# Sagnac/OpticalRayTracing.jl

Measured on NVIDIA B200. Metric: FP64 ray-surface intersections/sec, higher is better.
Workload: dtype f64

## Files before the change

### opticalraytracing.jl_b200/csrc/kern_trace3d.cu

```cuda
#include "kern.cuh"

struct Hit {
    double xs, ys;
    double xf, yf;
    unsigned flags;
    double opl;
};

__device__ __forceinline__ double strict_opl_start(const RayS& r, int mode, double n0, double y, double x, double z0)
{
    if (mode == 1) return SD(SM(n0, -z0), r.k3);
    return SM(n0, SA(SM(x, r.k1), SM(y, r.k2)));
}

__device__ __forceinline__ double strict_opl_close(const RayS& r, const ort_field& f, double nlast)
{
    if (f.opd_radius == 0.0) return r.opl;
    const double qx = SS(r.x, f.opd_xc), qy = SS(r.y, f.opd_yc);
    const double b = SA(SM(qx, r.k1), SM(qy, r.k2));
    const double cq = SS(SA(SM(qx, qx), SM(qy, qy)), SM(f.opd_radius, f.opd_radius));
    const double sg = (f.opd_radius < 0.0) ? -1.0 : 1.0;
    const double tau = SS(-b, SM(sg, SQ(SS(SM(b, b), cq))));
    return SA(r.opl, SM(nlast, tau));
}

template <bool EXT, class SurfArray, bool POLY, bool XF>
__device__ __forceinline__ Hit trace_strict_impl(const SurfArray& S, int nsurf, int stop, double y, double x, double u, double v,
                                                 const ort_field* fld, double n0, double nlast, bool vignette, const double* poly,
                                                 int npoly, int* bad)
{
    RayS r;
    strict_init<XF>(r, y, x, u, v);
    if (EXT) r.opl = strict_opl_start(r, fld->mode, n0, y, x, fld->z0);
    Hit h; h.xs = h.ys = CUDART_NAN; h.opl = 0.0;
    for (int i = 0; i < nsurf; i++) {
        strict_step<EXT, POLY, XF>(S[i], r, vignette, (POLY && poly) ? poly + (size_t)i * npoly : nullptr, npoly);
        if (i == stop - 1) { h.xs = r.x; h.ys = r.y; }
    }
    h.xf = r.x; h.yf = r.y; h.flags = r.flags;
    if (EXT) h.opl = strict_opl_close(r, *fld, nlast);
    if (XF) *bad = r.bad;
    return h;
}

template <bool EXT, class SurfArray, bool POLY = false>
__device__ __forceinline__ Hit trace_strict(const SurfArray& S, int nsurf, int stop,
                                            double y, double x, double u, double v,
                                            const ort_field* fld = nullptr, double n0 = 1.0, double nlast = 1.0,
                                            bool vignette = false, const double* poly = nullptr, int npoly = 0)
{
    return trace_strict_impl<EXT, SurfArray, POLY, false>(S, nsurf, stop, y, x, u, v, fld, n0, nlast, vignette, poly, npoly, nullptr);
}

template <bool EXT, class SurfArray, bool POLY = false>
__device__ __noinline__ Hit trace_strict_cold(const SurfArray& S, int nsurf, int stop,
                                              double y, double x, double u, double v,
                                              const ort_field* fld = nullptr, double n0 = 1.0, double nlast = 1.0,
                                              bool vignette = false, const double* poly = nullptr, int npoly = 0)
{
    return trace_strict<EXT, SurfArray, POLY>(S, nsurf, stop, y, x, u, v, fld, n0, nlast, vignette, poly, npoly);
}

template <bool EXT, class SurfArray, bool POLY = false>
__device__ __forceinline__ Hit trace_strict_xf(const SurfArray& S, int nsurf, int stop,
                                               double y, double x, double u, double v,
                                               const ort_field* fld = nullptr, double n0 = 1.0, double nlast = 1.0,
                                               bool vignette = false, const double* poly = nullptr, int npoly = 0)
{
    int bad = 0;
    const Hit h = trace_strict_impl<EXT, SurfArray, POLY, true>(S, nsurf, stop, y, x, u, v, fld, n0, nlast, vignette, poly, npoly, &bad);
    if (bad) return trace_strict_cold<EXT, SurfArray, POLY>(S, nsurf, stop, y, x, u, v, fld, n0, nlast, vignette, poly, npoly);
    return h;
}

__device__ __forceinline__ int nonfinite_bit(double a) { return 0x7FEFFFFF - (hi32(a) & 0x7FFFFFFF); }

__device__ __forceinline__ bool is_nan_bits(double a)
{
    return (hi32(a) & 0x7FFFFFFF) > 0x7FF00000 ||
           ((hi32(a) & 0x7FFFFFFF) == 0x7FF00000 && __double2loint(a) != 0);
}

template <int RPT, bool EXT, class SurfArray, bool MIRROR = true, int SIMPLE = 0, bool R2ONLY = false, int POLY = 0, class QT = NoPolyK>
__device__ __forceinline__ void trace_fast(const SurfArray& S, int nsurf, int stop, double n0,
                                           const double* y, const double* x, const double* u,
                                           const double* v, Hit* h, int* amb,
                                           const ort_field* fld = nullptr, double nlast = 1.0, bool vignette = false,
                                           const double* K0 = nullptr, bool kzcheck = true, const double* poly = nullptr,
                                           int npoly = 0, const QT* Q = nullptr)
{
    RaysF<RPT> r;
#pragma unroll
    for (int j = 0; j < RPT; j++) {
        if (K0) {
            r.x[j] = x[j]; r.y[j] = y[j]; r.z[j] = 0.0;
            r.Kx[j] = K0[0]; r.Ky[j] = K0[1]; r.Kz[j] = K0[2];
            r.amb[j] = 0; r.opl[j] = 0.0; r.vig[j] = 0;
        } else fast_init(r, j, n0, y[j], x[j], u[j], v[j]);
        if (EXT) {
            r.opl[j] = (fld->mode == 1) ? fast_div(-(n0 * n0) * fld->z0, r.Kz[j]) : fma(x[j], r.Kx[j], y[j] * r.Ky[j]);
        }
    }
    int i = 0;
    for (; i < stop; i++)
        if constexpr (POLY == 2) fast_step<RPT, EXT, MIRROR, SIMPLE, 2>(S[i], r, vignette, nullptr, 0, 0, &Q->r[i]);
        else fast_step<RPT, EXT, MIRROR, SIMPLE, POLY>(S[i], r, vignette, (POLY && poly) ? poly + (size_t)i * npoly : nullptr, npoly, nsurf * npoly);
#pragma unroll
    for (int j = 0; j < RPT; j++) {
        if (R2ONLY) { h[j].xs = fma(r.x[j], r.x[j], r.y[j] * r.y[j]); h[j].ys = 0.0; }
        else { h[j].xs = r.x[j]; h[j].ys = r.y[j]; }
    }
    for (; i < nsurf; i++)
        if constexpr (POLY == 2) fast_step<RPT, EXT, MIRROR, SIMPLE, 2>(S[i], r, vignette, nullptr, 0, 0, &Q->r[i]);
        else fast_step<RPT, EXT, MIRROR, SIMPLE, POLY>(S[i], r, vignette, (POLY && poly) ? poly + (size_t)i * npoly : nullptr, npoly, nsurf * npoly);
#pragma unroll
    for (int j = 0; j < RPT; j++) {
        h[j].xf = r.x[j]; h[j].yf = r.y[j];
        h[j].flags = (EXT && r.vig[j]) ? ORT_FLAG_VIGN : 0u;
        amb[j] = r.amb[j] | nonfinite_bit(r.x[j]) | nonfinite_bit(r.y[j]);
        if (kzcheck) amb[j] |= nonfinite_bit(r.Kz[j]);
        h[j].opl = 0.0;
        if (EXT) {
            double opl = r.opl[j];
            if (fld->opd_radius != 0.0) {
                const double qx = r.x[j] - fld->opd_xc, qy = r.y[j] - fld->opd_yc;
                const double bK = fma(qx, r.Kx[j], qy * r.Ky[j]);
                const double cq = fma(qx, qx, fma(qy, qy, -fld->opd_radius * fld->opd_radius));
                const double d = fma(bK, bK, -(nlast * nlast) * cq);
                double sq = fast_sqrt(d);
                if ((fld->opd_radius < 0.0) != (nlast < 0.0)) sq = -sq;
                opl = opl - bK - sq;
                amb[j] |= nonfinite_bit(opl);
            }
            h[j].opl = opl;
        }
    }
}

struct RawAcc {
    int n, nflag_lo, nflag_hi;
    double s1x, s2x, s1y, s2y, rmax;
    double s1o, s2o; int nvig;
    int nstrict;
};

__device__ __forceinline__ void raw_add(RawPart& p, const RawPart& q)
{
    p.n += q.n; p.s1x += q.s1x; p.s2x += q.s2x; p.s1y += q.s1y; p.s2y += q.s2y;
    p.rmax = fmax(p.rmax, q.rmax);
    p.nmiss += q.nmiss; p.ntir += q.ntir; p.ndom += q.ndom; p.nclip += q.nclip;
    p.s1o += q.s1o; p.s2o += q.s2o; p.nvig += q.nvig; p.nstrict += q.nstrict;
}

__device__ __forceinline__ void raw_warp_reduce(RawPart& p)
{
#pragma unroll
    for (int d = 16; d >= 1; d >>= 1) {
        p.n += __shfl_down_sync(0xffffffffu, p.n, d);
        p.s1x += __shfl_down_sync(0xffffffffu, p.s1x, d);
        p.s2x += __shfl_down_sync(0xffffffffu, p.s2x, d);
        p.s1y += __shfl_down_sync(0xffffffffu, p.s1y, d);
        p.s2y += __shfl_down_sync(0xffffffffu, p.s2y, d);
        p.rmax = fmax(p.rmax, __shfl_down_sync(0xffffffffu, p.rmax, d));
        p.nmiss += __shfl_down_sync(0xffffffffu, p.nmiss, d);
        p.ntir += __shfl_down_sync(0xffffffffu, p.ntir, d);
        p.ndom += __shfl_down_sync(0xffffffffu, p.ndom, d);
        p.nclip += __shfl_down_sync(0xffffffffu, p.nclip, d);
        p.s1o += __shfl_down_sync(0xffffffffu, p.s1o, d);
        p.s2o += __shfl_down_sync(0xffffffffu, p.s2o, d);
        p.nvig += __shfl_down_sync(0xffffffffu, p.nvig, d);
        p.nstrict += __shfl_down_sync(0xffffffffu, p.nstrict, d);
    }
}

template <int NWARPS>
__device__ __forceinline__ void raw_block_reduce(RawPart& p, RawPart* smem )
{
    raw_warp_reduce(p);
    const int lane = threadIdx.x & 31, warp = threadIdx.x >> 5;
    if (lane == 0) smem[warp] = p;
    __syncthreads();
    if (threadIdx.x == 0)
        for (int w = 1; w < NWARPS; w++) raw_add(p, smem[w]);
}

__device__ __forceinline__ void field_slopes(const ort_field& fld, double y0, double x0, double& u, double& v)
{
    u = fld.u; v = fld.v;
    if (fld.mode == 1) {
        u = tan(SD(SS(fld.ybar, y0), fld.z0));
        v = tan(SD(-x0, fld.z0));
    }
}

struct LeanPtrs { double *ex, *ey, *opd; uint8_t* mask; };
template <int ARITH, int EXTK, int LEAN, bool R2ONLY = false, int POLYK = 0>
__device__ __forceinline__ int grid_epilogue(const Presc& P, const GridArgs& A, const ort_field& fld,
                                             const double* ysf, Hit h, int amb, unsigned idx,
                                             bool valid, size_t fbase, double cx, double cy, double co, RawAcc& acc,
                                             const LeanPtrs& lp)
{
    constexpr bool EXT = EXTK != 0;
    const size_t o = fbase + idx;
    const bool vignette = EXTK == 1 && (A.ext & ORT_EXT_VIGNETTE);
    double ri = 0.0, r2 = 0.0;
    bool clip = false;
    if (ARITH == ORT_ARITH_FAST) {
        r2 = R2ONLY ? h.xs : fma(h.xs, h.xs, h.ys * h.ys);
        amb |= tiny_vs_bit(r2 - A.a_stop2, A.a_stop2);
        clip = r2 > A.a_stop2;
    }
    const bool sv = (ARITH == ORT_ARITH_STRICT) || amb < 0;
    if (sv) {
        if (ARITH != ORT_ARITH_STRICT) {
            const unsigned iy = idx / (unsigned)A.nx, ix = idx - iy * (unsigned)A.nx;
            const double y0 = __ldg(ysf + iy), x0 = __ldg(A.xs + ix);
            double u, v; field_slopes(fld, y0, x0, u, v);
            h = trace_strict_cold<EXT, decltype(P.s), POLYK != 0>(P.s, P.nsurf, A.stop, y0, x0, u, v, &fld, P.n0, P.nlast, vignette, P.poly, P.npoly);
        }
        ri = jl_hypot(h.xs, h.ys);
        clip = ri > A.a_stop;
        r2 = ri * ri;
        if (valid) {
            acc.nstrict++;
            acc.nflag_lo += (h.flags & ORT_FLAG_MISS ? 1 : 0) + (h.flags & ORT_FLAG_TIR ? 0x10000 : 0);
            acc.nflag_hi += (h.flags & ORT_FLAG_DOMAIN ? 1 : 0);
        }
    } else if (!LEAN && A.r) {
        ri = (r2 > 0.0) ? fast_sqrt(r2) : r2;
    }
    const bool vig = EXTK == 1 && (h.flags & ORT_FLAG_VIGN);
    const bool drop = clip || vig || (sv && (is_nan_bits(h.xf) || is_nan_bits(h.yf)));
    const unsigned flags = h.flags | (clip ? ORT_FLAG_CLIP : 0u);
    const int kept = valid && !drop;
    const double ex = h.xf;
    const double ey = SS(h.yf, fld.h_prime);
    double opd = 0.0;
    if (EXT && (A.ext & ORT_EXT_OPD)) opd = SM(SS(h.opl, fld.opl_ref), A.opd_scale);
    if (LEAN) {
        if (valid) {
            if (LEAN == 1) { *lp.ex = ex; *lp.ey = ey; *lp.mask = (uint8_t)kept; }
            if (LEAN == 1 && EXT) *lp.opd = opd;
            if (EXTK == 1) acc.nvig += vig ? 1 : 0;
            if (clip) acc.nflag_hi += 0x10000;
        }
    } else if (valid) {
        if (A.ex) A.ex[o] = ex;
        if (A.ey) A.ey[o] = ey;
        if (A.r) A.r[o] = ri;
        if (A.theta) A.theta[o] = atan2(h.ys, h.xs);
        if (A.wx) A.wx[o] = SD(SM(ex, A.wg_nu), A.wg_lambda);
        if (A.wy) A.wy[o] = SD(SM(ey, A.wg_nu), A.wg_lambda);
        if (EXT && A.opd) A.opd[o] = opd;
        if (A.mask) A.mask[o] = (uint8_t)kept;
        if (A.flags) A.flags[o] = (uint8_t)flags;
        acc.nflag_hi += clip ? 0x10000 : 0;
        if (EXT) acc.nvig += vig ? 1 : 0;
    }
    if (kept) {
        const double dx = ex - cx, dy = ey - cy;
        acc.s1x += dx; acc.s2x = fma(dx, dx, acc.s2x);
        acc.s1y += dy; acc.s2y = fma(dy, dy, acc.s2y);
        { const double rv = (ARITH == ORT_ARITH_STRICT) ? ri : r2; if (rv > acc.rmax) acc.rmax = rv; }
        if (EXT) { const double dd = opd - co; acc.s1o += dd; acc.s2o = fma(dd, dd, acc.s2o); }
        acc.n++;
    }
    return kept;
}

template <int ARITH, int RPT, int EXTK, int LEAN = 0, bool MIRROR = true, int SIMPLE = 0, int POLYK = 0>
__global__ void __launch_bounds__(ORT_TILE, (ARITH == ORT_ARITH_FAST) ? POLYK ? ORT_BPS_POLY : (SIMPLE == 2 ? ORT_BPSC : SIMPLE ? (EXTK ? ORT_BPSE : ORT_BPSP) : (RPT == 1 ? ORT_BPS1 : (EXTK ? ORT_BPS2E : ORT_BPS2))) : ORT_BPSS)
k_grid(const __grid_constant__ Presc P, const __grid_constant__ GridArgs A, const __grid_constant__ typename PolyArg<POLYK>::type Q)
{
    constexpr bool EXT = EXTK != 0;
    __shared__ RawPart s_part[ORT_TILE / 32];
    __shared__ double s_shift[3];
    const int f = blockIdx.y;
    const ort_field& fld = A.fields[f];
    const unsigned NN = A.NN;
    const unsigned nsub = (NN + ORT_TILE - 1) / ORT_TILE;
    const unsigned ntiles = (nsub + RPT - 1) / RPT;
    const size_t fbase = (size_t)f * NN;
    const double* ysf = A.ys + (size_t)f * A.ys_stride;
    const unsigned ysoff = (unsigned)f * (unsigned)A.ys_stride;
    const bool vignette = EXTK == 1 && (A.ext & ORT_EXT_VIGNETTE);

    RawAcc acc;
    acc.n = acc.nflag_lo = acc.nflag_hi = acc.nvig = acc.nstrict = 0;
    acc.s1x = acc.s2x = acc.s1y = acc.s2y = acc.s1o = acc.s2o = 0.0; acc.rmax = -CUDART_INF;

    if (threadIdx.x == 0) {
        const double y0 = __ldg(ysf + A.ny / 2), x0 = __ldg(A.xs);
        double u, v; field_slopes(fld, y0, x0, u, v);
        Hit h; int amb = 0;
        if (ARITH == ORT_ARITH_FAST)
            trace_fast<1, EXT, decltype(P.s), SIMPLE == 0, SIMPLE, false, POLYK, typename PolyArg<POLYK>::type>(P.s, P.nsurf, A.stop, P.n0, &y0, &x0, &u, &v, &h, &amb, &fld, P.nlast, vignette,
                                                                   nullptr, true, P.poly, P.npoly, &Q);
        if (ARITH == ORT_ARITH_STRICT || amb < 0)
            h = trace_strict_cold<EXT, decltype(P.s), (EXT && ARITH == ORT_ARITH_STRICT) || POLYK != 0>(P.s, P.nsurf, A.stop, y0, x0, u, v, &fld, P.n0,
                                                                                                  P.nlast, vignette, P.poly, P.npoly);
        const double ey = h.yf - fld.h_prime;
        const bool bad = nonfinite_bit(h.xf) < 0 || nonfinite_bit(ey) < 0;
        s_shift[0] = bad ? 0.0 : h.xf;
        s_shift[1] = bad ? 0.0 : ey;
        const double od = (h.opl - fld.opl_ref) * A.opd_scale;
        s_shift[2] = (!EXT || !(A.ext & ORT_EXT_OPD) || bad || nonfinite_bit(od) < 0) ? 0.0 : od;
    }
    __syncthreads();
    const double cx = s_shift[0], cy = s_shift[1], co = s_shift[2];
    constexpr bool R2ONLY = ARITH == ORT_ARITH_FAST && LEAN != 0;
    const bool kzcheck = P.s[P.nsurf - 1].kcode != SURF_PLANE;

    const bool collimated = (fld.mode == 0);
    double K0[3] = {0.0, 0.0, 0.0};
    if (ARITH == ORT_ARITH_FAST && collimated) {
        const double inv = P.n0 * fast_rsqrt(fma(fld.v, fld.v, fma(fld.u, fld.u, 1.0)));
        K0[0] = fld.v * inv; K0[1] = fld.u * inv; K0[2] = inv;
    }
    const unsigned nxu = (unsigned)A.nx;
    const unsigned step = gridDim.x * (RPT * ORT_TILE);
    const unsigned dq = step / nxu, dr = step - dq * nxu;
    unsigned iyj[RPT], ixj[RPT];
#pragma unroll
    for (int j = 0; j < RPT; j++) {
        const unsigned i0 = (blockIdx.x * RPT + j) * ORT_TILE + threadIdx.x;
        iyj[j] = i0 / nxu; ixj[j] = i0 - iyj[j] * nxu;
    }

    for (unsigned tile = blockIdx.x; tile < ntiles; tile += gridDim.x) {
        double y0[RPT], x0[RPT], u[RPT], v[RPT];
        unsigned idx[RPT];
        bool valid[RPT];
#pragma unroll
        for (int j = 0; j < RPT; j++) {
            const unsigned i0 = (tile * RPT + j) * ORT_TILE + threadIdx.x;
            valid[j] = i0 < NN;
            idx[j] = min(i0, NN - 1);
            const unsigned iy = min(iyj[j], (unsigned)A.ny - 1), ix = ixj[j];
            y0[j] = __ldg(A.ys + (ysoff + iy)); x0[j] = __ldg(A.xs + ix);
            u[j] = 0.0; v[j] = 0.0;
            ixj[j] += dr; iyj[j] += dq;
            if (ixj[j] >= nxu) { ixj[j] -= nxu; iyj[j]++; }
        }
        if (!collimated || ARITH != ORT_ARITH_FAST) {
#pragma unroll
            for (int j = 0; j < RPT; j++) field_slopes(fld, y0[j], x0[j], u[j], v[j]);
        }
        Hit h[RPT];
        int amb[RPT];
        if (ARITH == ORT_ARITH_FAST)
            trace_fast<RPT, EXT, decltype(P.s), MIRROR, SIMPLE, R2ONLY, POLYK, typename PolyArg<POLYK>::type>(P.s, P.nsurf, A.stop, P.n0, y0, x0, u, v, h, amb, &fld, P.nlast, vignette,
                                                                collimated ? K0 : nullptr, kzcheck, P.poly, P.npoly, &Q);
        else {
            RayS r[RPT];
#pragma unroll
            for (int j = 0; j < RPT; j++) {
                strict_init<ORT_STRICT_XF>(r[j], y0[j], x0[j], u[j], v[j]);
                if (EXT) r[j].opl = strict_opl_start(r[j], fld.mode, P.n0, y0[j], x0[j], fld.z0);
                h[j].xs = h[j].ys = CUDART_NAN; h[j].opl = 0.0;
            }
            const int nsurf = P.nsurf, stop = A.stop;
            for (int i = 0; i < nsurf; i++) {
#pragma unroll
                for (int j = 0; j < RPT; j++) {
                    strict_step<EXT, EXT, ORT_STRICT_XF>(P.s[i], r[j], vignette, (EXT && P.poly) ? P.poly + (size_t)i * P.npoly : nullptr, P.npoly);
                    if (i == stop - 1) { h[j].xs = r[j].x; h[j].ys = r[j].y; }
                }
            }
#pragma unroll
            for (int j = 0; j < RPT; j++) {
                h[j].xf = r[j].x; h[j].yf = r[j].y; h[j].flags = r[j].flags;
                if (EXT) h[j].opl = strict_opl_close(r[j], fld, P.nlast);
                if (ORT_STRICT_XF && r[j].bad)
                    h[j] = trace_strict_cold<EXT, decltype(P.s), EXT>(P.s, P.nsurf, A.stop, y0[j], x0[j], u[j], v[j], &fld, P.n0, P.nlast, vignette, P.poly, P.npoly);
            }
        }
        int keptj[RPT];
        LeanPtrs lp0 = {nullptr, nullptr, nullptr, nullptr};
        if (LEAN == 1) {
            const size_t e0 = fbase + (size_t)tile * (RPT * ORT_TILE) + threadIdx.x;
            lp0.ex = A.ex + e0; lp0.ey = A.ey + e0; lp0.mask = A.mask + e0;
            if (EXT) lp0.opd = A.opd + e0;
        }
#pragma unroll
        for (int j = 0; j < RPT; j++) {
            if (ARITH != ORT_ARITH_FAST) amb[j] = 0;
            const LeanPtrs lp = {lp0.ex + j * ORT_TILE, lp0.ey + j * ORT_TILE, EXT ? lp0.opd + j * ORT_TILE : nullptr, lp0.mask + j * ORT_TILE};
            keptj[j] = grid_epilogue<ARITH, EXTK, LEAN, R2ONLY, POLYK>(P, A, fld, ysf, h[j], amb[j], idx[j], valid[j],
                                                                fbase, cx, cy, co, acc, lp);
        }
        if (LEAN != 2 && A.tile_counts) {
#pragma unroll
            for (int j = 0; j < RPT; j++) {
                const int c = __syncthreads_count(keptj[j]);
                const unsigned sub = tile * RPT + j;
                if (threadIdx.x == 0 && sub < nsub) A.tile_counts[(size_t)f * nsub + sub] = c;
            }
        }
    }
    RawPart p;
    p.n = acc.n; p.s1x = acc.s1x; p.s2x = acc.s2x; p.s1y = acc.s1y; p.s2y = acc.s2y; p.rmax = acc.rmax;
    p.cx = cx; p.cy = cy; p.co = co; p.s1o = acc.s1o; p.s2o = acc.s2o; p.nvig = acc.nvig; p.nstrict = acc.nstrict;
    p.nmiss = acc.nflag_lo & 0xFFFF; p.ntir = acc.nflag_lo >> 16; p.ndom = acc.nflag_hi & 0xFFFF; p.nclip = acc.nflag_hi >> 16;
    raw_block_reduce<ORT_TILE / 32>(p, s_part);
    if (threadIdx.x == 0) {
        if (ARITH != ORT_ARITH_STRICT) p.rmax = sqrt(p.rmax);
        A.partials[(size_t)f * gridDim.x + blockIdx.x] = p;
    }
}

__global__ void __launch_bounds__(256) k_grid_finalize(const RawPart* partials, int nparts, ort_stats* stats)
{
    __shared__ RawPart s_part[8];
    const int f = blockIdx.x;
    RawPart p;
    p.n = 0; p.s1x = p.s2x = p.s1y = p.s2y = p.s1o = p.s2o = 0.0; p.rmax = -CUDART_INF; p.cx = p.cy = p.co = 0.0;
    p.nmiss = p.ntir = p.ndom = p.nclip = p.nvig = p.nstrict = 0;
    for (int j = threadIdx.x; j < nparts; j += 256) raw_add(p, partials[(size_t)f * nparts + j]);
    raw_block_reduce<8>(p, s_part);
    if (threadIdx.x == 0) {
        const RawPart& p0 = partials[(size_t)f * nparts];
        ort_stats s;
        s.n_kept = p.n;
        if (p.n > 0) {
            const double n = (double)p.n;
            s.mean_x = p0.cx + p.s1x / n; s.mean_y = p0.cy + p.s1y / n;
            s.m2_x = fmax(p.s2x - p.s1x * p.s1x / n, 0.0);
            s.m2_y = fmax(p.s2y - p.s1y * p.s1y / n, 0.0);
            s.r_max = p.rmax;
            s.mean_opd = p0.co + p.s1o / n;
            s.m2_opd = fmax(p.s2o - p.s1o * p.s1o / n, 0.0);
        } else { s.mean_x = s.mean_y = s.m2_x = s.m2_y = s.mean_opd = s.m2_opd = 0.0; s.r_max = -CUDART_INF; }
        s.n_miss = p.nmiss; s.n_tir = p.ntir; s.n_domain = p.ndom; s.n_clip = p.nclip; s.n_vig = p.nvig; s.n_strict = p.nstrict;
        stats[f] = s;
    }
}

#define SCAN_CHUNK 2048
__global__ void __launch_bounds__(256) k_tile_scan(int* counts, int* chunk_tot, unsigned ntiles, unsigned nchunks)
{
    __shared__ int s_warp[8];
    const unsigned f = blockIdx.y, chunk = blockIdx.x;
    int* c = counts + (size_t)f * ntiles + (size_t)chunk * SCAN_CHUNK;
    const unsigned n = min((unsigned)SCAN_CHUNK, ntiles - chunk * SCAN_CHUNK);
    const unsigned base = threadIdx.x * 8;
    int v[8], sum = 0;
#pragma unroll
    for (int j = 0; j < 8; j++) { v[j] = (base + j < n) ? c[base + j] : 0; sum += v[j]; }
    const int lane = threadIdx.x & 31, warp = threadIdx.x >> 5;
    int incl = sum;
#pragma unroll
    for (int d = 1; d < 32; d <<= 1) { int t = __shfl_up_sync(0xffffffffu, incl, d); if (lane >= d) incl += t; }
    if (lane == 31) s_warp[warp] = incl;
    __syncthreads();
    int woff = 0, tot = 0;
    for (int w = 0; w < 8; w++) { if (w < warp) woff += s_warp[w]; tot += s_warp[w]; }
    int run = woff + incl - sum;
#pragma unroll
    for (int j = 0; j < 8; j++) { if (base + j < n) c[base + j] = run; run += v[j]; }
    if (threadIdx.x == 0) chunk_tot[(size_t)f * nchunks + chunk] = tot;
}

__global__ void __launch_bounds__(256) k_chunk_scan(int* chunk_tot, unsigned nchunks)
{
    __shared__ int s_warp[8];
    int* c = chunk_tot + (size_t)blockIdx.x * nchunks;
    int carry = 0;
    for (unsigned base0 = 0; base0 < nchunks; base0 += 256) {
        const unsigned i = base0 + threadIdx.x;
        const int v = (i < nchunks) ? c[i] : 0;
        const int lane = threadIdx.x & 31, warp = threadIdx.x >> 5;
        int incl = v;
#pragma unroll
        for (int d = 1; d < 32; d <<= 1) { int t = __shfl_up_sync(0xffffffffu, incl, d); if (lane >= d) incl += t; }
        if (lane == 31) s_warp[warp] = incl;
        __syncthreads();
        int woff = 0, tot = 0;
        for (int w = 0; w < 8; w++) { if (w < warp) woff += s_warp[w]; tot += s_warp[w]; }
        if (i < nchunks) c[i] = carry + woff + incl - v;
        carry += tot;
        __syncthreads();
    }
}

__device__ __forceinline__ int compact_offset(const CompactArgs& C, unsigned tile, unsigned f, unsigned ntiles, unsigned tid,
                                              int m)
{
    __shared__ int s_warp[ORT_TILE / 32];
    const unsigned ball = __ballot_sync(0xffffffffu, m);
    const int lane = tid & 31, warp = tid >> 5;
    if (lane == 0) s_warp[warp] = __popc(ball);
    __syncthreads();
    int off = C.tile_offsets[(size_t)f * ntiles + tile];
    {
        const unsigned nchunks = (ntiles + SCAN_CHUNK - 1) / SCAN_CHUNK, mychunk = tile / SCAN_CHUNK;
        const int* ct = C.tile_offsets + (size_t)gridDim.y * ntiles + (size_t)f * nchunks;
        off += ct[mychunk];
    }
    for (int w = 0; w < warp; w++) off += s_warp[w];
    return off + __popc(ball & ((1u << lane) - 1u));
}

__global__ void __launch_bounds__(ORT_TILE) k_compact(CompactArgs C)
{
    const unsigned tile = blockIdx.x, f = blockIdx.y;
    const unsigned ntiles = (C.NN + ORT_TILE - 1) / ORT_TILE;
    const unsigned i = tile * ORT_TILE + threadIdx.x;
    const size_t fbase = (size_t)f * C.NN;
    const int m = (i < C.NN) ? C.mask[fbase + i] : 0;
    const int off = compact_offset(C, tile, f, ntiles, threadIdx.x, m);
    if (m) {
#pragma unroll
        for (int a = 0; a < 7; a++)
            if (C.src[a]) C.dst[a][fbase + off] = C.src[a][fbase + i];
    }
}

struct FocusRay {
    double a0, a1, a2, a3, a4, a5;
};

__device__ __forceinline__ void focus_pos_strict(const FocusRay& q, double t, double& xf, double& yf)
{
    const double ti = SS(t, q.a2);
    double y = SA(q.a1, SM(q.a4, ti));
    double x = SA(q.a0, SM(q.a3, ti));
    y = SA(y, SM(0.0, q.a4));
    x = SA(x, SM(0.0, q.a3));
    xf = x; yf = y;
}

__device__ __forceinline__ void focus_pos_fast(const FocusRay& q, double t, double& xf, double& yf)
{
    const double s = (t - q.a2) * q.a5;
    xf = fma(s, q.a3, q.a0);
    yf = fma(s, q.a4, q.a1);
}

__device__ __forceinline__ double fast_div_rcp(double d)
{
    double r = mufu_rcp(d);
    const double e = fma(-d, r, 1.0);
    return fma(r, fma(e, e, e), r);
}

struct FocusS {
    FocusRay q;
    double xs, ys;
    unsigned flags;
};

#define FOCUS_TIR_LAST 0x80u

template <bool XF>
__device__ __forceinline__ FocusS focus_strict_impl(const Presc& P, int stop, double y, double x, double u, double v, int* bad)
{
    RayS r;
    strict_init<XF>(r, y, x, u, v);
    FocusS o; o.xs = o.ys = CUDART_NAN;
    const int ns = P.nsurf - 1;
    for (int i = 0; i < ns; i++) {
        strict_step<false, false, XF>(P.s[i], r);
        if (i == stop - 1) { o.xs = r.x; o.ys = r.y; }
    }
    const SurfK& S = P.s[ns];
    double dot = SA(0.0, SM(r.k1, 0.0)); dot = SA(dot, SM(r.k2, 0.0)); dot = SA(dot, SM(r.k3, -1.0));
    const double gam = -dot;
    const double Dr = SS(1.0, SM(S.etasq, SS(1.0, SM(gam, gam))));
    if (Dr < 0.0) r.flags |= FOCUS_TIR_LAST;
    o.q.a0 = r.x; o.q.a1 = r.y; o.q.a2 = r.sprev; o.q.a3 = r.v; o.q.a4 = r.u; o.q.a5 = 0.0;
    o.flags = r.flags;
    if (XF) *bad = r.bad;
    return o;
}

__device__ __noinline__ FocusS focus_strict_cold(const Presc& P, int stop, double y, double x, double u, double v)
{
    return focus_strict_impl<false>(P, stop, y, x, u, v, nullptr);
}

template <int ARITH, int RPT, bool MIRROR, int SIMPLE>
__global__ void __launch_bounds__(ORT_TILE, 2)
k_focus(const __grid_constant__ Presc P, const __grid_constant__ FocusArgs F)
{
    constexpr int NWARPS = ORT_TILE / 32;
    __shared__ double s_acc[NWARPS][ORT_MAX_FOCI][4];
    __shared__ double s_c[ORT_MAX_FOCI][2];
    __shared__ RawPart s_part[NWARPS];
    __shared__ RawPart s_p0;
    __shared__ double2 s_xy[RPT][ORT_TILE];
    __shared__ int s_cnt[4][ORT_TILE];
    __shared__ double s_rmax[ORT_TILE];
    const GridArgs& A = F.G;
    const int M = F.n_foci;
    const int f = blockIdx.y;
    const ort_field& fld = A.fields[f];
    const unsigned NN = A.NN;
    const unsigned nsub = (NN + ORT_TILE - 1) / ORT_TILE;
    const unsigned ntiles = (nsub + RPT - 1) / RPT;
    const size_t fbase = (size_t)f * NN;
    const double* ysf = A.ys + (size_t)f * A.ys_stride;
    const unsigned ysoff = (unsigned)f * (unsigned)A.ys_stride;
    const int lane = threadIdx.x & 31, warp = threadIdx.x >> 5;

    for (int i = threadIdx.x; i < NWARPS * ORT_MAX_FOCI * 4; i += ORT_TILE) (&s_acc[0][0][0])[i] = 0.0;
    if (threadIdx.x == 0) {
        const double y0 = __ldg(ysf + A.ny / 2), x0 = __ldg(A.xs);
        double u, v; field_slopes(fld, y0, x0, u, v);
        const FocusS c = focus_strict_cold(P, A.stop, y0, x0, u, v);
        for (int m = 0; m < M; m++) {
            double xf, yf; focus_pos_strict(c.q, F.foci[m], xf, yf);
            const double ey = yf - fld.h_prime;
            const bool bad = nonfinite_bit(xf) < 0 || nonfinite_bit(ey) < 0;
            s_c[m][0] = bad ? 0.0 : xf;
            s_c[m][1] = bad ? 0.0 : ey;
        }
    }
    __syncthreads();

    int* const cnt_n = &s_cnt[0][threadIdx.x];
    int* const cnt_lo = &s_cnt[1][threadIdx.x];
    int* const cnt_hi = &s_cnt[2][threadIdx.x];
    int* const cnt_strict = &s_cnt[3][threadIdx.x];
    *cnt_n = *cnt_lo = *cnt_hi = *cnt_strict = 0;
    s_rmax[threadIdx.x] = -CUDART_INF;
    const SurfK& SL = P.s[P.nsurf - 1];
    const bool refr_last = (SL.kcode & SURF_REFR) != 0;
    const bool collimated = (fld.mode == 0);
    double K0[3] = {0.0, 0.0, 0.0};
    if (ARITH == ORT_ARITH_FAST && collimated) {
        const double inv = P.n0 * fast_rsqrt(fma(fld.v, fld.v, fma(fld.u, fld.u, 1.0)));
        K0[0] = fld.v * inv; K0[1] = fld.u * inv; K0[2] = inv;
    }
    const unsigned nxu = (unsigned)A.nx;

    for (unsigned tile = blockIdx.x; tile < ntiles; tile += gridDim.x) {
        double y0[RPT], x0[RPT], u[RPT], v[RPT];
        unsigned idx[RPT];
        bool valid[RPT];
#pragma unroll
        for (int j = 0; j < RPT; j++) {
            const unsigned i0 = (tile * RPT + j) * ORT_TILE + threadIdx.x;
            valid[j] = i0 < NN;
            idx[j] = min(i0, NN - 1);
            const unsigned iy = idx[j] / nxu, ix = idx[j] - iy * nxu;
            y0[j] = __ldg(A.ys + (ysoff + iy)); x0[j] = __ldg(A.xs + ix);
            u[j] = 0.0; v[j] = 0.0;
        }
        if (!collimated || ARITH != ORT_ARITH_FAST) {
#pragma unroll
            for (int j = 0; j < RPT; j++) field_slopes(fld, y0[j], x0[j], u[j], v[j]);
        }
        FocusRay q[RPT];
        double xs[RPT], ys[RPT];
        unsigned flg[RPT];
        bool sv[RPT];
        if (ARITH == ORT_ARITH_FAST) {
            RaysF<RPT> r;
#pragma unroll
            for (int j = 0; j < RPT; j++) {
                if (collimated) {
                    r.x[j] = x0[j]; r.y[j] = y0[j]; r.z[j] = 0.0;
                    r.Kx[j] = K0[0]; r.Ky[j] = K0[1]; r.Kz[j] = K0[2];
                    r.amb[j] = 0; r.opl[j] = 0.0; r.vig[j] = 0;
                } else fast_init(r, j, P.n0, y0[j], x0[j], u[j], v[j]);
            }
            const int ns = P.nsurf - 1;
            int i = 0;
            for (; i < A.stop; i++) fast_step<RPT, false, MIRROR, SIMPLE, 0>(P.s[i], r);
#pragma unroll
            for (int j = 0; j < RPT; j++) s_xy[j][threadIdx.x] = make_double2(r.x[j], r.y[j]);
            for (; i < ns; i++) fast_step<RPT, false, MIRROR, SIMPLE, 0>(P.s[i], r);
#pragma unroll
            for (int j = 0; j < RPT; j++) {
                int amb = r.amb[j];
                if (refr_last) {
                    const double Dp = fma(r.Kz[j], r.Kz[j], SL.dn2);
                    amb |= hi32(Dp) - SL.tir_thr;
                    amb |= nonfinite_bit(MIRROR ? sign_of_n2(fast_sqrt(Dp), SL.n2mask) : fast_sqrt(Dp));
                }
                q[j].a0 = r.x[j]; q[j].a1 = r.y[j]; q[j].a2 = r.z[j]; q[j].a3 = r.Kx[j]; q[j].a4 = r.Ky[j];
                q[j].a5 = fast_div_rcp(r.Kz[j]);
                double xa, ya, xb, yb;
                focus_pos_fast(q[j], F.t_lo, xa, ya);
                focus_pos_fast(q[j], F.t_hi, xb, yb);
                amb |= nonfinite_bit(xa) | nonfinite_bit(ya) | nonfinite_bit(xb) | nonfinite_bit(yb);
                const double2 st = s_xy[j][threadIdx.x];
                const double r2 = fma(st.x, st.x, st.y * st.y);
                amb |= tiny_vs_bit(r2 - A.a_stop2, A.a_stop2);
                sv[j] = amb < 0;
                flg[j] = 0u;
            }
// ... 751 lines not shown
```

Measured before the change: 404.5 billion.

## Hoist strict fallback out of grid epilogue behind warp vote and specialize full tiles

Moves the rare strict re-trace fallback out of the per-ray epilogue into a block guarded by a warp-level any vote, so the common fast path avoids the inlined cold trace code and its register pressure. Full tiles skip bounds clamping and validity checks through compile-time specialized lambdas. The Kz finiteness check is folded into a branchless bit expression, and clip counting uses shifts. This adds code duplication and changes where index stepping happens, with some risk of subtle mismatch in the validity or output-index logic.

Result: no change. 407.0 billion (median of 6 runs) (+0.6%).

```diff
diff --git a/opticalraytracing.jl_b200/csrc/kern_trace3d.cu b/opticalraytracing.jl_b200/csrc/kern_trace3d.cu
--- a/opticalraytracing.jl_b200/csrc/kern_trace3d.cu
+++ b/opticalraytracing.jl_b200/csrc/kern_trace3d.cu
@@ -1,3 +1,5 @@
+#include <type_traits>
+
 #include "kern.cuh"
 
 struct Hit {
@@ -113,12 +115,12 @@
     for (; i < nsurf; i++)
         if constexpr (POLY == 2) fast_step<RPT, EXT, MIRROR, SIMPLE, 2>(S[i], r, vignette, nullptr, 0, 0, &Q->r[i]);
         else fast_step<RPT, EXT, MIRROR, SIMPLE, POLY>(S[i], r, vignette, (POLY && poly) ? poly + (size_t)i * npoly : nullptr, npoly, nsurf * npoly);
+    const int kzmask = kzcheck ? 0x7FFFFFFF : 0;
 #pragma unroll
     for (int j = 0; j < RPT; j++) {
         h[j].xf = r.x[j]; h[j].yf = r.y[j];
         h[j].flags = (EXT && r.vig[j]) ? ORT_FLAG_VIGN : 0u;
-        amb[j] = r.amb[j] | nonfinite_bit(r.x[j]) | nonfinite_bit(r.y[j]);
-        if (kzcheck) amb[j] |= nonfinite_bit(r.Kz[j]);
+        amb[j] = r.amb[j] | nonfinite_bit(r.x[j]) | nonfinite_bit(r.y[j]) | (0x7FEFFFFF - (hi32(r.Kz[j]) & kzmask));
         h[j].opl = 0.0;
         if (EXT) {
             double opl = r.opl[j];
@@ -194,45 +196,30 @@
 }
 
 struct LeanPtrs { double *ex, *ey, *opd; uint8_t* mask; };
-template <int ARITH, int EXTK, int LEAN, bool R2ONLY = false, int POLYK = 0>
-__device__ __forceinline__ int grid_epilogue(const Presc& P, const GridArgs& A, const ort_field& fld,
-                                             const double* ysf, Hit h, int amb, unsigned idx,
-                                             bool valid, size_t fbase, double cx, double cy, double co, RawAcc& acc,
-                                             const LeanPtrs& lp)
+
+__device__ __forceinline__ void strict_finish(const GridArgs& A, const Hit& h, bool valid, double& ri, double& r2,
+                                              int& clip, int& keep, RawAcc& acc)
+{
+    ri = jl_hypot(h.xs, h.ys);
+    clip = ri > A.a_stop;
+    r2 = ri * ri;
+    keep = !clip && !is_nan_bits(h.xf) && !is_nan_bits(h.yf);
+    if (valid) {
+        acc.nstrict++;
+        acc.nflag_lo += (h.flags & ORT_FLAG_MISS ? 1 : 0) + (h.flags & ORT_FLAG_TIR ? 0x10000 : 0);
+        acc.nflag_hi += (h.flags & ORT_FLAG_DOMAIN ? 1 : 0);
+    }
+}
+
+template <int ARITH, int EXTK, int LEAN>
+__device__ __forceinline__ int grid_epilogue(const GridArgs& A, const ort_field& fld, const Hit& h, double r2, double ri,
+                                             int clip, int keep, bool valid, size_t o, double cx, double cy, double co,
+                                             RawAcc& acc, const LeanPtrs& lp)
 {
     constexpr bool EXT = EXTK != 0;
-    const size_t o = fbase + idx;
-    const bool vignette = EXTK == 1 && (A.ext & ORT_EXT_VIGNETTE);
-    double ri = 0.0, r2 = 0.0;
-    bool clip = false;
-    if (ARITH == ORT_ARITH_FAST) {
-        r2 = R2ONLY ? h.xs : fma(h.xs, h.xs, h.ys * h.ys);
-        amb |= tiny_vs_bit(r2 - A.a_stop2, A.a_stop2);
-        clip = r2 > A.a_stop2;
-    }
-    const bool sv = (ARITH == ORT_ARITH_STRICT) || amb < 0;
-    if (sv) {
-        if (ARITH != ORT_ARITH_STRICT) {
-            const unsigned iy = idx / (unsigned)A.nx, ix = idx - iy * (unsigned)A.nx;
-            const double y0 = __ldg(ysf + iy), x0 = __ldg(A.xs + ix);
-            double u, v; field_slopes(fld, y0, x0, u, v);
-            h = trace_strict_cold<EXT, decltype(P.s), POLYK != 0>(P.s, P.nsurf, A.stop, y0, x0, u, v, &fld, P.n0, P.nlast, vignette, P.poly, P.npoly);
-        }
-        ri = jl_hypot(h.xs, h.ys);
-        clip = ri > A.a_stop;
-        r2 = ri * ri;
-        if (valid) {
-            acc.nstrict++;
-            acc.nflag_lo += (h.flags & ORT_FLAG_MISS ? 1 : 0) + (h.flags & ORT_FLAG_TIR ? 0x10000 : 0);
-            acc.nflag_hi += (h.flags & ORT_FLAG_DOMAIN ? 1 : 0);
-        }
-    } else if (!LEAN && A.r) {
-        ri = (r2 > 0.0) ? fast_sqrt(r2) : r2;
-    }
     const bool vig = EXTK == 1 && (h.flags & ORT_FLAG_VIGN);
-    const bool drop = clip || vig || (sv && (is_nan_bits(h.xf) || is_nan_bits(h.yf)));
     const unsigned flags = h.flags | (clip ? ORT_FLAG_CLIP : 0u);
-    const int kept = valid && !drop;
+    const int kept = (valid && !vig) ? keep : 0;
     const double ex = h.xf;
     const double ey = SS(h.yf, fld.h_prime);
     double opd = 0.0;
@@ -242,7 +229,7 @@
             if (LEAN == 1) { *lp.ex = ex; *lp.ey = ey; *lp.mask = (uint8_t)kept; }
             if (LEAN == 1 && EXT) *lp.opd = opd;
             if (EXTK == 1) acc.nvig += vig ? 1 : 0;
-            if (clip) acc.nflag_hi += 0x10000;
+            acc.nflag_hi += clip << 16;
         }
     } else if (valid) {
         if (A.ex) A.ex[o] = ex;
@@ -254,7 +241,7 @@
         if (EXT && A.opd) A.opd[o] = opd;
         if (A.mask) A.mask[o] = (uint8_t)kept;
         if (A.flags) A.flags[o] = (uint8_t)flags;
-        acc.nflag_hi += clip ? 0x10000 : 0;
+        acc.nflag_hi += clip << 16;
         if (EXT) acc.nvig += vig ? 1 : 0;
     }
     if (kept) {
@@ -327,21 +314,20 @@
         iyj[j] = i0 / nxu; ixj[j] = i0 - iyj[j] * nxu;
     }
 
+    const unsigned nfull = NN / (RPT * ORT_TILE);
     for (unsigned tile = blockIdx.x; tile < ntiles; tile += gridDim.x) {
+        const bool full = tile < nfull;
         double y0[RPT], x0[RPT], u[RPT], v[RPT];
-        unsigned idx[RPT];
-        bool valid[RPT];
-#pragma unroll
-        for (int j = 0; j < RPT; j++) {
-            const unsigned i0 = (tile * RPT + j) * ORT_TILE + threadIdx.x;
-            valid[j] = i0 < NN;
-            idx[j] = min(i0, NN - 1);
-            const unsigned iy = min(iyj[j], (unsigned)A.ny - 1), ix = ixj[j];
-            y0[j] = __ldg(A.ys + (ysoff + iy)); x0[j] = __ldg(A.xs + ix);
-            u[j] = 0.0; v[j] = 0.0;
-            ixj[j] += dr; iyj[j] += dq;
-            if (ixj[j] >= nxu) { ixj[j] -= nxu; iyj[j]++; }
-        }
+        auto load_xy = [&](auto full_t) {
+#pragma unroll
+            for (int j = 0; j < RPT; j++) {
+                const unsigned iy = decltype(full_t)::value ? iyj[j] : min(iyj[j], (unsigned)A.ny - 1), ix = ixj[j];
+                y0[j] = __ldg(A.ys + (ysoff + iy)); x0[j] = __ldg(A.xs + ix);
+                u[j] = 0.0; v[j] = 0.0;
+            }
+        };
+        if (full) load_xy(std::true_type());
+        else load_xy(std::false_type());
         if (!collimated || ARITH != ORT_ARITH_FAST) {
 #pragma unroll
             for (int j = 0; j < RPT; j++) field_slopes(fld, y0[j], x0[j], u[j], v[j]);
@@ -375,19 +361,59 @@
                     h[j] = trace_strict_cold<EXT, decltype(P.s), EXT>(P.s, P.nsurf, A.stop, y0[j], x0[j], u[j], v[j], &fld, P.n0, P.nlast, vignette, P.poly, P.npoly);
             }
         }
-        int keptj[RPT];
+        double r2[RPT], ri[RPT];
+        int clip[RPT], keep[RPT];
+        if (ARITH == ORT_ARITH_FAST) {
+            int need = 0;
+#pragma unroll
+            for (int j = 0; j < RPT; j++) {
+                r2[j] = R2ONLY ? h[j].xs : fma(h[j].xs, h[j].xs, h[j].ys * h[j].ys);
+                amb[j] |= tiny_vs_bit(r2[j] - A.a_stop2, A.a_stop2);
+                clip[j] = r2[j] > A.a_stop2;
+                keep[j] = !clip[j];
+                ri[j] = 0.0;
+                if (!LEAN && A.r) ri[j] = (r2[j] > 0.0) ? fast_sqrt(r2[j]) : r2[j];
+                need |= amb[j];
+            }
+            if (__any_sync(0xffffffffu, need < 0)) {
+#pragma unroll
+                for (int j = 0; j < RPT; j++) {
+                    if (amb[j] >= 0) continue;
+                    const unsigned i0 = (tile * RPT + j) * ORT_TILE + threadIdx.x, idx = min(i0, NN - 1);
+                    const unsigned iy = idx / nxu, ix = idx - iy * nxu;
+                    const double ys = __ldg(ysf + iy), xs = __ldg(A.xs + ix);
+                    double us, vs; field_slopes(fld, ys, xs, us, vs);
+                    h[j] = trace_strict_cold<EXT, decltype(P.s), POLYK != 0>(P.s, P.nsurf, A.stop, ys, xs, us, vs, &fld, P.n0, P.nlast, vignette, P.poly, P.npoly);
+                    strict_finish(A, h[j], i0 < NN, ri[j], r2[j], clip[j], keep[j], acc);
+                }
+            }
+        } else {
+#pragma unroll
+            for (int j = 0; j < RPT; j++)
+                strict_finish(A, h[j], (tile * RPT + j) * ORT_TILE + threadIdx.x < NN, ri[j], r2[j], clip[j], keep[j], acc);
+        }
+        const size_t e0 = fbase + (size_t)tile * (RPT * ORT_TILE) + threadIdx.x;
         LeanPtrs lp0 = {nullptr, nullptr, nullptr, nullptr};
         if (LEAN == 1) {
-            const size_t e0 = fbase + (size_t)tile * (RPT * ORT_TILE) + threadIdx.x;
             lp0.ex = A.ex + e0; lp0.ey = A.ey + e0; lp0.mask = A.mask + e0;
             if (EXT) lp0.opd = A.opd + e0;
         }
+        int keptj[RPT];
+        auto epilogue = [&](auto full_t) {
+#pragma unroll
+            for (int j = 0; j < RPT; j++) {
+                const bool valid = decltype(full_t)::value || (tile * RPT + j) * ORT_TILE + threadIdx.x < NN;
+                const LeanPtrs lp = {lp0.ex + j * ORT_TILE, lp0.ey + j * ORT_TILE, EXT ? lp0.opd + j * ORT_TILE : nullptr, lp0.mask + j * ORT_TILE};
+                keptj[j] = grid_epilogue<ARITH, EXTK, LEAN>(A, fld, h[j], r2[j], ri[j], clip[j], keep[j], valid,
+                                                           e0 + j * ORT_TILE, cx, cy, co, acc, lp);
+            }
+        };
+        if (LEAN != 0 && full) epilogue(std::true_type());
+        else epilogue(std::false_type());
 #pragma unroll
         for (int j = 0; j < RPT; j++) {
-            if (ARITH != ORT_ARITH_FAST) amb[j] = 0;
-            const LeanPtrs lp = {lp0.ex + j * ORT_TILE, lp0.ey + j * ORT_TILE, EXT ? lp0.opd + j * ORT_TILE : nullptr, lp0.mask + j * ORT_TILE};
-            keptj[j] = grid_epilogue<ARITH, EXTK, LEAN, R2ONLY, POLYK>(P, A, fld, ysf, h[j], amb[j], idx[j], valid[j],
-                                                                fbase, cx, cy, co, acc, lp);
+            ixj[j] += dr; iyj[j] += dq;
+            if (ixj[j] >= nxu) { ixj[j] -= nxu; iyj[j]++; }
         }
         if (LEAN != 2 && A.tile_counts) {
 #pragma unroll
```
